# mjoppich/tsxCount

Hardware: AMD Instinct MI355X
Metric: k-mers/sec inserted, k=31, 1e9 synthetic k-mers, 1/2/4/8 GPU; --check pass (higher is better)
Workload: dtype u64

## Files before the change

### tsxcount_amd/csrc/tsx_partition.h

```cpp
#pragma once
#include "tsx_kernels.h"
#include "tsx_layout.h"
#include <type_traits>

namespace tsx {

constexpr int PART_NT = 256;
constexpr int RING_NT = 512;
constexpr int PART_WPT = 4;
constexpr int PART_FLUSH = 16;

template <int RW>
__device__ __forceinline__ void load_rec(const uint64_t *ptr, uint64_t (&r)[RW]) {
    if constexpr (RW == 1) {
        r[0] = *ptr;
    } else {
#pragma unroll
        for (int t = 0; t < RW; t += 2) {
            const uint4 v = *reinterpret_cast<const uint4 *>(ptr + t);
            r[t] = (uint64_t)v.x | ((uint64_t)v.y << 32);
            r[t + 1] = (uint64_t)v.z | ((uint64_t)v.w << 32);
        }
    }
}
template <int RW>
__device__ __forceinline__ void store_rec(uint64_t *ptr, const uint64_t (&r)[RW]) {
    if constexpr (RW == 1) {
        *ptr = r[0];
    } else {
#pragma unroll
        for (int t = 0; t < RW; t += 2)
            *reinterpret_cast<uint4 *>(ptr + t) = make_uint4((uint32_t)r[t], (uint32_t)(r[t] >> 32), (uint32_t)r[t + 1],
                                                             (uint32_t)(r[t + 1] >> 32));
    }
}

constexpr uint32_t OVF_N = 64;
constexpr uint64_t OVF_SALT = 0x5DEECE66D1CE4E5BULL;

__device__ __forceinline__ uint64_t format_record(const TableParams &p, uint64_t key) {
    const uint32_t q1 = ((uint32_t)key + 1u) & (uint32_t)p.seg_mask;
    return ((key >> p.lg) << p.R) | ((uint64_t)q1 << (p.R + p.F));
}

constexpr int PART_MAX_PIECES = 512;
constexpr int PART_ITER = 3;
template <int RW> struct SpillState {
    static constexpr uint32_t DCH_MAX = (RW == 4) ? 48 : 96;
    uint64_t ovk[OVF_N * RW];
    unsigned long long dch[DCH_MAX];
    uint32_t ovc[OVF_N];
    uint32_t ovr[OVF_N];
    uint32_t ovn;
    uint32_t dn;
    uint32_t skew;
};
#define TSX_LDS __attribute__((address_space(3)))
template <int RW>
__device__ __forceinline__ void spill_record(const TableParams *pk, TSX_LDS SpillState<RW> *sp, uint64_t *ovq, uint32_t ovq_cap,
                                             uint32_t dch, RecVal<RW> r, uint32_t d) {
    sp->skew = 1u;
    const uint64_t kk = r.w[0] ^ OVF_SALT;
    if (kk != 0) {
// ... 367 lines not shown
                    if (homeless) spill(cur[q]);
                }
            }
        };
        if constexpr (SKEW) {
            if (s_sp.skew != 0u) append(std::true_type{});
            else append(std::false_type{});
        } else {
            append(std::false_type{});
        }
        lds_barrier();
        flush(false, [&]() {
            __builtin_amdgcn_s_waitcnt(0x0F70);
#pragma unroll
            for (int q = 0; q < RPT; ++q)
#pragma unroll
                for (int t = 0; t < RW; ++t) cur[q][t] = nxt[q][t];
        });
        lds_barrier();
        bc = bn;
    }
    flush(true, []() {});
    lds_barrier();
    {
        const uint32_t dn = SKEW ? s_sp.dn : 0u;
        if (dch && dn % dch != 0u && (dn - 1u) / dch < SpillState<RW>::DCH_MAX) {
            const unsigned long long first = s_sp.dch[(dn - 1u) / dch] - 1ULL;
            if (first + dch <= pk->defer.cap)
                for (uint32_t o = dn % dch + tid; o < dch; o += NT) pk->defer.cnt[first + o] = 0ULL;
        }
    }
    if (dst_cnt)
        for (uint32_t b = tid; b < nb; b += NT) {
            const uint64_t li = dst_bm ? ((uint64_t)b * dst_nr + dst_r0 + r) * cpr + c : ((uint64_t)r * nb + b) * cpr + c;
            dst_cnt[li] = (min(s_cur[b], s_lim[b]) - li * dst_cap * RW) / RW;
        }
    if (tid < OVF_N && s_sp.ovc[tid]) {
        uint64_t rec[RW];
#pragma unroll
        for (int t = 0; t < RW; ++t) rec[t] = s_sp.ovk[tid * RW + t];
        rec[0] ^= OVF_SALT;
        defer_append<RW>(pk, rec, s_sp.ovc[tid]);
    }
    if (tid == 0 && ovq_cnt) ovq_cnt[blockIdx.x] = min(s_sp.ovn, ovq_cap);
    for (int d = 32; d > 0; d >>= 1) spilled += __shfl_down(spilled, d, 64);
    if ((tid & 63) == 0 && spilled) atomicAdd(&p.stats[ST_FALLBACK], (unsigned long long)spilled);
    if (key_sum) {
        for (int d = 32; d > 0; d >>= 1) ksum += __shfl_down(ksum, d, 64);
        if ((tid & 63) == 0 && ksum) atomicAdd(key_sum, ksum);
    }
}

constexpr int SP_NT = 512;
constexpr uint32_t SP_CAPBITS = 5;

__global__ __launch_bounds__(1024) void desc_prefix_kernel(const unsigned long long *cnt, uint32_t nregions,
                                                           unsigned long long *offs, unsigned long long *total,
                                                           uint64_t desc_cap, uint64_t out_cap, unsigned long long *stats) {
    __shared__ unsigned long long s_w[16];
    const uint32_t tid = threadIdx.x, per = (nregions + 1023u) / 1024u;
    unsigned long long sum = 0, lost = 0;
    for (uint32_t i = 0; i < per; ++i) {
        const uint32_t r = tid * per + i;
        if (r < nregions) { sum += min((unsigned long long)cnt[r], (unsigned long long)desc_cap); lost += cnt[r] > desc_cap ? cnt[r] - desc_cap : 0ULL; }
    }
    const unsigned long long inc = wave_incl_scan64(sum);
    if ((tid & 63) == 63) s_w[tid >> 6] = inc;
    __syncthreads();
    unsigned long long base = inc - sum;
    for (uint32_t w = 0; w < (tid >> 6); ++w) base += s_w[w];
    for (uint32_t i = 0; i < per; ++i) {
        const uint32_t r = tid * per + i;
        if (r < nregions) { offs[r] = base; base += min((unsigned long long)cnt[r], (unsigned long long)desc_cap); }
    }
    if (lost && stats) atomicAdd(&stats[ST_FAIL], lost);
    if (tid == 1023) {
        if (base > out_cap) { if (stats) atomicAdd(&stats[ST_FAIL], base - out_cap); base = out_cap; }
        total[0] = base;
    }
}
__global__ __launch_bounds__(256) void desc_pack_kernel(const uint4 *desc, uint64_t desc_cap, const unsigned long long *cnt,
                                                        const unsigned long long *offs, uint32_t nregions, uint4 *out,
                                                        uint64_t out_cap, uint32_t du) {
    for (uint32_t r = blockIdx.x; r < nregions; r += gridDim.x) {
        const uint64_t n = min((uint64_t)cnt[r], desc_cap) * du, o = offs[r] * du;
        const uint4 *src = desc + (uint64_t)r * desc_cap * du;
        for (uint64_t i = threadIdx.x; i < n; i += 256)
            if (o + i < out_cap) out[o + i] = src[i];
    }
}

template <int NT, bool CANON = false, bool LOCAL = false>
__global__ __launch_bounds__(NT, 4) void walk_part_kernel(TableParams p, const uint4 *desc, uint64_t desc_cap,
                                                            const unsigned long long *desc_cnt, uint32_t nregions,
                                                            uint64_t *dst, uint64_t dst_cap, unsigned long long *dst_cnt,
                                                            uint32_t nb, uint32_t shift, uint64_t *ovq_all,
                                                            uint32_t *ovq_cnt, uint32_t ovq_cap, uint64_t n_packed,
                                                            uint32_t dst_g0, uint32_t dst_gtot, int own_flags,
                                                            unsigned long long *emit_sum, int long_desc, uint32_t flush_q,
                                                            int dst_wgm) {
    const int own_only = LOCAL ? 0 : own_flags & 3;
    const bool append = !LOCAL && (own_flags & 4) != 0;
    if constexpr (LOCAL) { n_packed = 0; dst_g0 = 0; long_desc = 0; }
    constexpr int HOT_N = 8;
    __shared__ uint64_t s_hot_key[(NT / 64) * HOT_N];
    __shared__ uint32_t s_hot_cnt[(NT / 64) * HOT_N];
    __shared__ uint64_t s_roll[CANON ? 128 : 64];
    __shared__ uint64_t s_lut4[256];
    uint64_t *const s_mroll = s_roll + 64;
    __shared__ uint64_t s_homh[4];
    __shared__ uint32_t s_njobs[2];
    __shared__ uint32_t s_ovn;
    __shared__ uint64_t s_ovk[OVF_N];
    __shared__ uint32_t s_ovc[OVF_N];
    extern __shared__ uint64_t s_part[];
    constexpr uint32_t CAP = 1u << SP_CAPBITS, cmask = CAP - 1;
    uint64_t *s_stage = s_part;
    unsigned long long *s_meta = reinterpret_cast<unsigned long long *>(s_part + ((size_t)nb << SP_CAPBITS));
    unsigned long long *s_th = s_meta + nb;
    uint32_t *s_cur = reinterpret_cast<uint32_t *>(s_th + nb);
    uint32_t *s_job = s_cur + nb;

    const uint32_t tid = threadIdx.x, lane = tid & 63, wave = tid >> 6;
    const uint32_t wg = blockIdx.x;
    const uint32_t cap32 = (uint32_t)min(dst_cap, (uint64_t)0xFFFFFFF0u);
    const uint32_t gl = dst_g0 + wg;
    const SubListOrder ord = sublist_order(nb, dst_gtot, dst_wgm);
    const uint32_t li0 = sublist_number(ord, 0, gl);
    auto word_of = [&](uint32_t b, uint32_t at) -> uint64_t * { return dst + ((uint64_t)(li0 + b * ord.step_b) * (uint64_t)cap32 + at); };
    auto is_mine = [&](uint64_t hk) -> bool {
        if constexpr (LOCAL) return true;
        if (own_only != 1) return true;
        const uint64_t h1[1] = {hk};
        return owner_shard<1>(p, h1) == p.shard;
    };
    if (tid < 64) s_roll[tid] = p.roll[tid];
    if (tid < 256) s_lut4[tid] = p.roll[64 + tid];
    if (CANON && tid < 64) s_mroll[tid] = p.roll[MROLL1_AT + tid];
    if (tid < 4) {
        const uint64_t x = (0x5555555555555555ULL * (uint64_t)tid) & p.top_mask;
        uint64_t hh = 0;
        for (int grp = 0; grp < 16; ++grp) hh ^= p.roll[64 + grp * 16 + ((x >> (4 * grp)) & 15u)];
        if constexpr (CANON) {
            const uint64_t xc = (0x5555555555555555ULL * (uint64_t)(3 - tid)) & p.top_mask;
            uint64_t hc = 0;
            for (int grp = 0; grp < 16; ++grp) hc ^= p.roll[64 + grp * 16 + ((xc >> (4 * grp)) & 15u)];
            hh = min(hh, hc);
        }
        s_homh[tid] = hh;
    }
    if (tid < (NT / 64) * HOT_N) { s_hot_key[tid] = 0; s_hot_cnt[tid] = 0; }
    if (tid < OVF_N) { s_ovk[tid] = 0; s_ovc[tid] = 0; }
    if (tid < 2) s_njobs[tid] = 0;
    if (tid == 0) s_ovn = (append && ovq_cnt) ? ovq_cnt[blockIdx.x] : 0u;
    for (uint32_t b = tid; b < nb; b += NT) { s_cur[b] = append ? (uint32_t)dst_cnt[li0 + b * ord.step_b] : 0u; s_th[b] = 0; }
    uint64_t *ovq = ovq_all ? ovq_all + (size_t)blockIdx.x * ovq_cap : nullptr;
    unsigned long long added = 0;
    unsigned long long emitted = 0;
    uint32_t spilled = 0;
    const uint32_t k = (uint32_t)p.k;
    const uint32_t inc_ws = (2u * k) >> 5, inc_sh = (2u * k) & 31u;
    const bool two_dwords = k > 16u;
    auto first_hash = [&](uint64_t x) -> uint64_t {
        const uint32_t xl = (uint32_t)x, xh = (uint32_t)(x >> 32);
        uint64_t hx = 0;
#pragma unroll
        for (int grp = 0; grp < 8; ++grp) hx ^= s_lut4[grp * 16 + __builtin_amdgcn_ubfe(xl, 4 * grp, 4)];
        if (two_dwords) {
#pragma unroll
            for (int grp = 0; grp < 8; ++grp) hx ^= s_lut4[128 + grp * 16 + __builtin_amdgcn_ubfe(xh, 4 * grp, 4)];
        }
// ... 6 lines not shown
        const uint64_t kk = key ^ OVF_SALT;
        if (kk != 0) {
            const uint32_t slot = (uint32_t)(mix64(key) >> 40) & (OVF_N - 1);
            const unsigned long long old = atomicCAS(reinterpret_cast<unsigned long long *>(&s_ovk[slot]), 0ULL,
                                                     (unsigned long long)kk);
            if (old == 0ULL || old == kk) { atomicAdd(&s_ovc[slot], 1u); return; }
        }
        if (ovq) {
            const uint32_t at = atomicAdd(&s_ovn, 1u);
            if (at < ovq_cap) { ovq[at] = key; return; }
        }
        defer_append1(pk, key, 1);
    };
    uint32_t round = 0;
    auto flush = [&](bool all, bool wait_loads) {
        const uint32_t par = round & 1u;
        ++round;
        if (tid == 0) s_njobs[par ^ 1u] = 0;
        for (uint32_t b = tid; b < nb; b += NT) {
            const unsigned long long th = s_th[b];
            const uint32_t head = (uint32_t)(th >> 32);
            const uint32_t tail = min((uint32_t)th, head + CAP);
            const uint32_t avail = tail - head;
            const uint32_t at = s_cur[b];
            const uint32_t end = (at + avail) & ~(uint32_t)(PART_FLUSH - 1);
            const uint32_t nout = all ? avail : (end > at ? end - at : 0u);
            s_meta[b] = ((unsigned long long)at << 16) | ((unsigned long long)(head & cmask) << 8) | nout;
            s_th[b] = ((unsigned long long)(head + nout) << 32) | tail;
            s_cur[b] = at + nout;
            if (nout) s_job[atomicAdd(&s_njobs[par], 1u)] = b;
        }
        lds_barrier();
        if (wait_loads) __builtin_amdgcn_s_waitcnt(0x0F70);
        const uint32_t oct = tid >> 3, ol = tid & 7;
        const uint32_t njobs = s_njobs[par];
        constexpr int ITER = 2;
        for (uint32_t j0 = 0; j0 < njobs; j0 += ITER * (NT / 8)) {
            unsigned long long meta[ITER];
            uint32_t bj[ITER];
            uint64_t k0[ITER], k1[ITER];
#pragma unroll
            for (int u = 0; u < ITER; ++u) {
                const uint32_t j = j0 + oct + u * (NT / 8);
                bj[u] = (j < njobs) ? s_job[j] : 0u;
            }
#pragma unroll
            for (int u = 0; u < ITER; ++u) {
                const uint32_t j = j0 + oct + u * (NT / 8);
                meta[u] = (j < njobs) ? s_meta[bj[u]] : 0ULL;
            }
#pragma unroll
            for (int u = 0; u < ITER; ++u) {
                const uint32_t nout = (uint32_t)meta[u] & 0xFFu, hd = ((uint32_t)meta[u] >> 8) & 0xFFu;
                const uint64_t *ring = s_stage + (bj[u] << SP_CAPBITS);
                k0[u] = (ol < nout) ? ring[((hd + ol) ^ bj[u]) & cmask] : 0;
                k1[u] = (ol + 8 < nout) ? ring[((hd + ol + 8) ^ bj[u]) & cmask] : 0;
            }
#pragma unroll
            for (int u = 0; u < ITER; ++u) {
                const uint32_t nout = (uint32_t)meta[u] & 0xFFu, hd = ((uint32_t)meta[u] >> 8) & 0xFFu;
                const uint32_t at = (uint32_t)(meta[u] >> 16);
                const uint64_t *ring = s_stage + (bj[u] << SP_CAPBITS);
                uint64_t *out = word_of(bj[u], at);
                if (ol < nout) { if (at + ol < cap32) out[ol] = k0[u]; else spill(k0[u]); }
                if (ol + 8 < nout) { if (at + ol + 8 < cap32) out[ol + 8] = k1[u]; else spill(k1[u]); }
                if (nout > 16)
                    for (uint32_t q = ol + 16; q < nout; q += 8) {
                        const uint64_t w = ring[((hd + q) ^ bj[u]) & cmask];
                        if (at + q < cap32) out[q] = w; else spill(w);
                    }
            }
        }
    };

    lds_barrier();
    for (uint32_t r = blockIdx.x; r < nregions; r += gridDim.x) {
        uint32_t nr;
        if constexpr (LOCAL) nr = (uint32_t)min((uint64_t)desc_cnt[r], desc_cap);
        else nr = n_packed ? (uint32_t)(((uint64_t)r * desc_cap < n_packed) ? min(desc_cap, n_packed - (uint64_t)r * desc_cap) : 0ULL)
                           : (uint32_t)min((uint64_t)desc_cnt[r], desc_cap);
        const uint32_t per = long_desc ? NT / 4 : NT, me = long_desc ? tid >> 2 : tid;
        const uint4 *rd = desc + (uint64_t)r * desc_cap * (long_desc ? 2u : 1u);
        const uint4 z4 = make_uint4(0, 0, 0, 0);
        uint4 dn = z4, dn2 = z4;
        if (me < nr) { if (long_desc) { dn = rd[2u * me]; dn2 = rd[2u * me + 1u]; } else dn = rd[me]; }
        for (uint32_t base = 0; base < nr; base += per) {
            const uint4 d = dn, d2 = dn2;
            if (base + per < nr) {
                dn = z4; dn2 = z4;
                if (base + per + me < nr) {
                    if (long_desc) { dn = rd[2u * (base + per + me)]; dn2 = rd[2u * (base + per + me) + 1u]; }
                    else dn = rd[base + per + me];
                }
            }
            uint32_t cw0 = d.x, cw1 = d.y, cw2 = d.z, vm = d.w & 0xFFFFu;
            if (!LOCAL && long_desc) {
                const uint32_t t = tid & 3u;
                const uint32_t w0 = d.x, w1 = d.y, w2 = d.z, w3 = d.w, w4 = d2.x, w5 = d2.y;
                cw0 = (t == 0u) ? w0 : (t == 1u) ? w1 : (t == 2u) ? w2 : w3;
                cw1 = (t == 0u) ? w1 : (t == 1u) ? w2 : (t == 2u) ? w3 : w4;
                cw2 = (t == 0u) ? w2 : (t == 1u) ? w3 : (t == 2u) ? w4 : w5;
                const uint32_t vw = (t < 2u) ? d2.z : d2.w;
                vm = (vw >> ((t & 1u) * 16u)) & 0xFFFFu;
            }
            const bool wave_has = __ballot(vm != 0u) != 0ULL;
            uint64_t h = 0, hr = 0;
            uint32_t inc = 0, single = 0;
            if (wave_has) {
                const uint64_t lo = (uint64_t)cw0 | ((uint64_t)cw1 << 32), hi = cw2;
                if (vm) {
                    const uint64_t x = lo & p.top_mask;
                    h = first_hash(x);
                    if constexpr (CANON) {
                        const uint64_t xa[1] = {x};
                        uint64_t r[1];
// ... 44 lines not shown
                        if constexpr (!LOCAL) emitted += tot;
                        const uint64_t key = s_homh[b];
                        uint64_t *hkey = s_hot_key + wave * HOT_N;
                        uint32_t *hcnt = s_hot_cnt + wave * HOT_N;
                        int at = -1;
                        for (int q = 0; q < HOT_N; ++q)
                            if (hcnt[q] && hkey[q] == key) { at = q; break; }
                        if (at < 0)
                            for (int q = 0; q < HOT_N; ++q)
                                if (!hcnt[q]) { at = q; hkey[q] = key; break; }
                        if (at >= 0 && (uint64_t)hcnt[at] + tot < 0xFFFFFFF0ULL) hcnt[at] += tot;
                        else defer_append1(pk, key, tot);
                    }
                }
            }
        }
            bool waited = false;
            for (uint32_t j0 = 0; j0 < 16; j0 += 4) {
                const uint32_t s4 = (single >> j0) & 0xFu;
                if (wave_has) {
                    uint64_t hs[4];
#pragma unroll
                    for (int j = 0; j < 4; ++j) {
                        hs[j] = CANON ? min(h, hr) : h;
                        if (j0 + j < 15) {
                            const uint32_t idx = ((uint32_t)h & 3u) | (__builtin_amdgcn_ubfe(cw0, 2u * (j0 + j), 2u) << 2) |
                                                 (__builtin_amdgcn_ubfe(inc, 2u * (j0 + j), 2u) << 4);
                            if constexpr (CANON) hr = mirror_step(p, s_mroll, hr, idx);
                            h = (h >> 2) ^ s_roll[idx];
                        }
                    }
                    uint32_t m4 = s4;
                    if constexpr (!LOCAL) if (own_only) {
                        if (own_only == 1) {
#pragma unroll
                            for (int j = 0; j < 4; ++j)
                                if (((s4 >> j) & 1u) && !is_mine(hs[j])) m4 &= ~(1u << j);
                        }
                        emitted += (unsigned long long)__popc(m4);
                    }
                    if (__ballot(m4 != 0u) != 0ULL) {
                        uint32_t bq[4];
                        unsigned long long sl[4];
#pragma unroll
                        for (int j = 0; j < 4; ++j) {
                            bq[j] = (uint32_t)(hs[j] >> shift) & (nb - 1);
                            sl[j] = ((m4 >> j) & 1u) ? atomicAdd(&s_th[bq[j]], 1ULL) : 0ULL;
                        }
#pragma unroll
                        for (int j = 0; j < 4; ++j) {
                            if ((m4 >> j) & 1u) {
                                const uint32_t b = bq[j];
                                if ((uint32_t)sl[j] - (uint32_t)(sl[j] >> 32) < CAP) {
                                    s_stage[(b << SP_CAPBITS) + (((uint32_t)sl[j] ^ b) & cmask)] = hs[j];
                                } else {
                                    const uint32_t at = atomicAdd(&s_cur[b], 1u);
                                    if (at < cap32) *word_of(b, at) = hs[j];
                                    else spill(hs[j]);
                                }
                            }
                        }
                    }
                }
                if (LOCAL || (((j0 >> 2) + 1u) % flush_q) == 0u) {
                    lds_barrier();
                    flush(false, !waited);
                    waited = true;
                    lds_barrier();
                }
            }
        }
    }
    lds_barrier();
    flush(true, false);
    lds_barrier();
    for (uint32_t b = tid; b < nb; b += NT) dst_cnt[li0 + b * ord.step_b] = min(s_cur[b], cap32);
    if (tid < OVF_N && s_ovc[tid]) defer_append1(pk, s_ovk[tid] ^ OVF_SALT, s_ovc[tid]);
    if (tid == 0 && ovq_cnt) ovq_cnt[blockIdx.x] = min(s_ovn, ovq_cap);
    if (tid < (NT / 64) * HOT_N && s_hot_cnt[tid]) defer_append1(pk, s_hot_key[tid], s_hot_cnt[tid]);
    if constexpr (!LOCAL) if (emit_sum) {
        for (int d = 32; d > 0; d >>= 1) emitted += __shfl_down(emitted, d, 64);
        if (lane == 0 && emitted) atomicAdd(emit_sum, emitted);
    }
    for (int d = 32; d > 0; d >>= 1) { added += __shfl_down(added, d, 64); spilled += __shfl_down(spilled, d, 64); }
    if (lane == 0) {
        if (added) atomicAdd(&p.stats[ST_KMERS], added);
        if (spilled) atomicAdd(&p.stats[ST_FALLBACK], (unsigned long long)spilled);
    }
}

inline bool walk_local_form(int own_flags, uint64_t n_packed, int long_desc, uint32_t flush_q, const void *emit_sum,
                            uint32_t dst_g0) {
    return own_flags == 0 && n_packed == 0 && !long_desc && flush_q == 1u && emit_sum == nullptr && dst_g0 == 0u;
}

template <int WK>
__global__ __launch_bounds__(PART_NT) void overflow_insert_kernel(TableParams p, const uint64_t *ovq_all,
                                                                  const uint32_t *ovq_cnt, uint32_t cap, uint32_t nq) {
    constexpr int RW = RecWords<WK>::value;
    for (uint32_t qi = blockIdx.x; qi < nq; qi += gridDim.x) {
        const uint32_t n = ovq_cnt[qi];
        for (uint32_t i = threadIdx.x; i < n; i += PART_NT) {
            uint64_t h[WK];
#pragma unroll
            for (int t = 0; t < WK; ++t) h[t] = ovq_all[((size_t)qi * cap + i) * RW + t];
            insert_key<WK>(p, h, 1);
        }
    }
}

template <int WK>
__global__ __launch_bounds__(PART_NT) void deferred_insert_kernel(TableParams p, const uint64_t *rec, const uint64_t *cnt,
                                                                  const unsigned long long *n_ptr, uint64_t n_fixed,
                                                                  uint64_t cap) {
    constexpr int RW = RecWords<WK>::value;
    const uint64_t n = min(n_ptr ? (uint64_t)*n_ptr : n_fixed, cap);
    constexpr uint32_t DN = (RW == 1) ? 2048u : (RW == 2) ? 1024u : 512u;
// ... 595 lines not shown
```

### tsxcount_amd/csrc/tsxcount_hip.hip

```cpp
#include "../../include/tsxcount_hip.h"
#include "tsx_kernels.h"
#include "tsx_partition.h"
#include "tsx_minimizer.h"
#include "tsx_inflate.h"
#include "tsx_output.h"
#include "tsx_query.h"
#include "tsx_baserule.h"
#include "tsx_db.h"
#include "tsx_combine.h"
#include "tsx_joint.h"
#include "tsx_het.h"
#include "tsx_bin.h"
#include "tsx_fasta.h"
#include "tsx_trim.h"
#include "tsx_normalize.h"
#include "tsx_sketch.h"
#include "tsx_prefilter.h"
#include "tsx_pairs.h"
#include "tsx_own.h"

#include <mutex>
#include <hip/hip_runtime.h>

#include <algorithm>
// ... 675 lines not shown
        case 2: { constexpr int WKV = 2; CALL; } break; \
        case 3: { constexpr int WKV = 3; CALL; } break; \
        default: { constexpr int WKV = 4; CALL; } break; \
    }
#define DISPATCH_CANON(m, CALL)                                                    \
    if ((m)->canon) { constexpr bool CANV = true; CALL; } else { constexpr bool CANV = false; CALL; }
#define DISPATCH_BR(m, CALL)                                                                                           \
    if ((m)->p.acgt_only || (m)->qmap_cur) { constexpr bool BRV = true; CALL; } else { constexpr bool BRV = false; CALL; }

static inline int rec_words(int wk) { return wk == 3 ? 4 : wk; }

static int max_seg_bits() {
    static int v = 0;
    if (!v) { v = 18; if (const char *e = getenv("TSX_HIP_SLAB_SEGBITS")) v = std::min(18, std::max(9, atoi(e))); }
    return v;
}
static int slab_bits(const tsx_hip_map *m) {
    const TableParams &p = m->p;
    const int nsegbits = p.l - p.S;
    if (nsegbits <= max_seg_bits() || p.wk != 1 || p.W != 1 || p.lg != p.l) return 0;
    return nsegbits - max_seg_bits();
}
static inline bool slab_build_wanted(const tsx_hip_map *m, size_t n) {
    return slab_bits(m) && (m->path == 2 || (m->path == 0 && n * 32 >= m->lay.table_bytes));
}
static bool can_partition(const tsx_hip_map *m) {
    const TableParams &p = m->p;
    const int nsegbits = p.l - p.S;
    if (nsegbits >= 1 && nsegbits <= (p.lg == p.l && p.wk == 1 && p.W == 1 ? max_seg_bits() : 18)) return true;
    const int sb = slab_bits(m);
    return sb >= 1 && sb <= 4;
}

struct RadixBits { int b1, b2; };
static inline RadixBits radix_bits(int nsegbits) {
    const int b1 = std::min(9, (nsegbits <= 8) ? nsegbits : (nsegbits + 1) / 2);
    return RadixBits{b1, nsegbits - b1};
}
static inline uint32_t cpr2_for(int cus, RadixBits rb) {
    if (rb.b2 <= 0) return 1;
    uint32_t c = std::min<uint32_t>(8, std::max<uint32_t>(1, (uint32_t)(cus * 8) / (1u << rb.b1)));
    while (c & (c - 1)) c &= c - 1;
    return c;
}
static uint32_t level2_cpr(const tsx_hip_map *m) { return cpr2_for(m->cus, radix_bits(m->p.l - m->p.S)); }
static inline uint32_t ring_bits(uint32_t nb) {
    const uint32_t mean = std::max<uint32_t>(1, RING_NT * PART_WPT / nb);
    uint32_t bits = 4;
    while ((1u << bits) < PART_FLUSH + 2 * mean && bits < 6) ++bits;
    return bits;
}
static const uint32_t RECV_RING_BITS = 5;
static inline size_t ring_lds_bytes(uint32_t nb, uint32_t bits) { return (size_t)nb * (((size_t)8 << bits) + 36); }
static inline size_t walk_lds_bytes(uint32_t nb1) { return (size_t)nb1 * (((size_t)8 << SP_CAPBITS) + 8 + 8 + 4 + 4); }
static const size_t ONE_WG_LDS = (size_t)80 << 10;

template <typename B>
static int grow(hipStream_t st, B &buf, size_t need) { return buf.reserve(&st, need, need + need / 8 + 4096); }

static int ensure_deferred(tsx_hip_map *m, uint64_t maxrec, hipStream_t st) {
    const int rw = rec_words(m->p.wk);
    if (!m->d_def_n.get()) TSX_TRY(m->d_def_n.alloc(64));
    if (maxrec > ((uint64_t)1 << 30)) maxrec = std::max<uint64_t>((uint64_t)1 << 28, maxrec / 16);
    if (maxrec <= m->def_cap()) return TSX_HIP_OK;
    const size_t cap = maxrec + maxrec / 8 + 4096;
    int rc = m->d_def_rec.reserve(&st, (size_t)maxrec * rw * 8, cap * rw * 8);
    if (rc == TSX_HIP_OK) rc = m->d_def_cnt.alloc(cap * 8);
    if (rc != TSX_HIP_OK) { m->d_def_rec.reset(); m->d_def_cnt.reset(); }
    return rc;
}

template <typename... K>
static int set_max_lds(int bytes, K... kernels) {
    for (const void *f : {(const void *)kernels...})
        HIP_TRY(hipFuncSetAttribute(f, hipFuncAttributeMaxDynamicSharedMemorySize, bytes));
    return TSX_HIP_OK;
}
template <int RW>
static int set_ring_lds(int bytes) {
    return set_max_lds(bytes, partition_ring_kernel<RW>, partition_ring_kernel<RW, 1024>, partition_ring_kernel<RW, RING_NT, true>,
                       partition_ring_kernel<RW, 1024, true>);
}
template <int NTV>
static int set_walk_lds(int bytes) {
    return set_max_lds(bytes, walk_part_kernel<NTV>, walk_part_kernel<NTV, true>, walk_part_kernel<NTV, false, true>,
                       walk_part_kernel<NTV, true, true>);
}
static int set_partition_attrs(tsx_hip_map *m) {
    if (m->attr_done) return TSX_HIP_OK;
    const int big = 150 << 10, seg = (128 << 10) + (32 << 10);
    TSX_TRY(set_ring_lds<1>(big)); TSX_TRY(set_ring_lds<2>(big)); TSX_TRY(set_ring_lds<4>(big));
    TSX_TRY(set_walk_lds<SP_NT>(big)); TSX_TRY(set_walk_lds<1024>(big));
    TSX_TRY(set_max_lds(seg, build_segments_stream_kernel<false>, build_segments_stream_kernel<true>,
                        build_segments_wide_stream_kernel<1>, build_segments_wide_stream_kernel<2>,
                        build_segments_wide_stream_kernel<3>, build_segments_wide_stream_kernel<4>));
    TSX_TRY(set_max_lds(64 << 10, walk_log_wide_kernel<3>, walk_log_wide_kernel<4>, walk_log_wide_kernel<3, true>,
                        walk_log_wide_kernel<4, true>));
    m->attr_done = true;
    return TSX_HIP_OK;
}

static int plan_partition(tsx_hip_map *m, uint64_t maxrec, int g, bool own_log, uint32_t hist_nb_override,
                          hipStream_t st, PartPlan &pl, int fused_g = 0) {
    const TableParams &p = m->p;
    const int nsegbits = p.l - p.S;
    pl.g = g;
    pl.rw = rec_words(p.wk);
    pl.nseg = 1u << nsegbits;
    const RadixBits rb = radix_bits(nsegbits);
    pl.b1 = rb.b1; pl.b2 = rb.b2;
    pl.nb1 = 1u << pl.b1; pl.nb2 = 1u << pl.b2;
    pl.hist_nb = hist_nb_override ? hist_nb_override : pl.nb1;
    auto even = [](uint64_t v) { return (v + 1) & ~1ULL; };
    pl.log_cap = even(maxrec / g + maxrec / g / 3 + 2048);
    if (const char *e = getenv("TSX_HIP_LOG_CAP")) pl.log_cap = even(std::max(16, atoi(e)));
    pl.cpr2 = cpr2_for(m->cus, rb);
    if (pl.b2) if (const char *e = getenv("TSX_HIP_CPR2")) pl.cpr2 = (uint32_t)std::min(8, std::max(1, atoi(e)));
    const uint64_t per_sub = maxrec / pl.nseg / pl.cpr2;
    pl.cap_sub = (per_sub + per_sub / 4 + 6 * (uint64_t)std::sqrt((double)per_sub + 1.0) + 64 + 15) & ~15ULL;
    pl.fused = fused_g > 0 && pl.b2 > 0 && p.wk == 1 && (fused_g + pl.cpr2 - 1) / pl.cpr2 <= (uint32_t)PART_MAX_PIECES;
    pl.G1 = pl.fused ? (uint32_t)fused_g : 0;
    pl.cap1 = 0;
    pl.l1_wgm = false;
    if (pl.fused) {
        const uint64_t per1 = maxrec / pl.nb1 / pl.G1;
        pl.cap1 = (per1 + per1 / 4 + 6 * (uint64_t)std::sqrt((double)per1 + 1.0) + 64 + 15) & ~15ULL;
        if (const char *e = getenv("TSX_HIP_CAP1")) pl.cap1 = (uint64_t)std::max(16, atoi(e) & ~15);
    }
    const uint64_t rec_cap = pl.fused ? 0 : (own_log ? (uint64_t)g * pl.log_cap : maxrec);
    const size_t need0 = std::max<uint64_t>(own_log ? rec_cap : 0, pl.b2 ? (uint64_t)pl.nseg * pl.cpr2 * pl.cap_sub : 0) * 8 * pl.rw;
    const size_t need1 = (pl.fused ? (uint64_t)pl.nb1 * pl.G1 * pl.cap1 : rec_cap) * 8 * pl.rw;
    TSX_TRY(grow(st, m->d_buf[0], need0));
    TSX_TRY(grow(st, m->d_buf[1], need1));
    pl.buf1 = m->d_buf[1].get();
    const uint32_t hb = std::max(pl.nb1, pl.hist_nb);
    pl.cnt_need = 2 * (size_t)g + 2 * (size_t)hb + (size_t)pl.nseg * pl.cpr2 + (size_t)pl.nb1 * pl.G1;
    const size_t mat = (size_t)hb * g;
    TSX_TRY(grow(st, m->d_cnt, pl.cnt_need * 8 + mat * 12 + 64));
    pl.c_log = m->d_cnt.get();
    pl.c_rstart = pl.c_log + g;
    pl.c_bstart = pl.c_rstart + g; pl.c_bcnt = pl.c_bstart + hb; pl.c_seg = pl.c_bcnt + hb;
    pl.c_l1 = pl.c_seg + (size_t)pl.nseg * pl.cpr2;
    pl.d_offs = pl.c_l1 + (size_t)pl.nb1 * pl.G1;
    pl.d_hist = reinterpret_cast<uint32_t *>(pl.d_offs + mat);
    HIP_TRY(hipMemsetAsync(m->d_cnt.get(), 0, pl.cnt_need * 8, st));
    TSX_TRY(set_partition_attrs(m));
    return TSX_HIP_OK;
}

struct WalkPartLaunch {
    uint32_t grid = 0;
    const uint4 *desc = nullptr; uint64_t desc_cap = 0; const unsigned long long *desc_cnt = nullptr; uint32_t nregions = 0;
    uint64_t *dst = nullptr; uint64_t dst_cap = 0; unsigned long long *dst_cnt = nullptr; uint32_t nb = 0, shift = 0;
    uint64_t *ovq_all = nullptr; uint32_t *ovq_cnt = nullptr; uint32_t ovq_cap = 0; uint64_t n_packed = 0;
    uint32_t dst_g0 = 0, dst_gtot = 0; int own_flags = 0; unsigned long long *emit_sum = nullptr; int long_desc = 0; uint32_t flush_q = 0;
    int dst_wgm = 0;
};
static void launch_walk_part(tsx_hip_map *m, hipStream_t st, const TableParams &pp, WalkPartLaunch &a) {
    const size_t lds = walk_lds_bytes(a.nb);
#define TSX_WALK(NTV, CANV, LOCV)                                                                                              \
    hipLaunchKernelGGL((walk_part_kernel<NTV, CANV, LOCV>), dim3(a.grid), dim3(NTV), lds, st, pp, a.desc, a.desc_cap,          \
                       a.desc_cnt, a.nregions, a.dst, a.dst_cap, a.dst_cnt, a.nb, a.shift, a.ovq_all, a.ovq_cnt, a.ovq_cap,    \
                       a.n_packed, a.dst_g0, a.dst_gtot, a.own_flags, a.emit_sum, a.long_desc, a.flush_q, a.dst_wgm)
    const bool local = walk_local_form(a.own_flags, a.n_packed, a.long_desc, a.flush_q, a.emit_sum, a.dst_g0);
    a.dst_wgm = local ? 1 : 0;
    if (lds > ONE_WG_LDS) {
        if (local) { DISPATCH_CANON(m, TSX_WALK(1024, CANV, true)); } else { DISPATCH_CANON(m, TSX_WALK(1024, CANV, false)); }
    } else {
        if (local) { DISPATCH_CANON(m, TSX_WALK(SP_NT, CANV, true)); } else { DISPATCH_CANON(m, TSX_WALK(SP_NT, CANV, false)); }
    }
#undef TSX_WALK
}

#define DISPATCH_RW(rw, CALL)                        \
    switch (rw) {                                    \
        case 1: { constexpr int RWV = 1; CALL; } break; \
        case 2: { constexpr int RWV = 2; CALL; } break; \
        default: { constexpr int RWV = 4; CALL; } break; \
    }

struct RingLaunch {
    uint32_t grid = 0;
    int rw = 1;
    bool skew = false;
    bool fixed_nt = false;
    const uint64_t *src = nullptr; const unsigned long long *src_start = nullptr, *src_cnt = nullptr; uint64_t src_cap = 0;
    uint32_t nregions = 0, cpr = 1; uint64_t *dst = nullptr; const unsigned long long *offs = nullptr, *offs_base = nullptr;
    unsigned long long *dst_cnt = nullptr; uint64_t dst_cap = 0; uint32_t nb = 0, shift = 0, capbits = 0;
    uint64_t *ovq_all = nullptr; uint32_t *ovq_cnt = nullptr; uint32_t ovq_cap = 0;
    const unsigned long long *src_pcnt = nullptr; uint32_t src_np = 0; uint64_t src_pcap = 0;
    int src_wgm = 0;
    int dst_bm = 0;
    unsigned long long *key_sum = nullptr; uint32_t dst_r0 = 0, dst_nr = 0; int fmt = 0; uint32_t dch = 0; const uint32_t *skew_flag = nullptr;
};
static void launch_ring(hipStream_t st, const TableParams &pp, const RingLaunch &a) {
    const size_t lds = ring_lds_bytes(a.nb, a.capbits);
#define TSX_RING(RWV, NTV, SK)                                                                                                 \
    hipLaunchKernelGGL((partition_ring_kernel<RWV, NTV, SK>), dim3(a.grid), dim3(NTV), lds, st, pp, a.src, a.src_start,        \
                       a.src_cnt, a.src_cap, a.nregions, a.cpr, a.dst, a.offs, a.offs_base, a.dst_cnt, a.dst_cap, a.nb,        \
                       a.shift, a.capbits, a.ovq_all, a.ovq_cnt, a.ovq_cap, a.src_pcnt, a.src_np, a.src_pcap, a.src_wgm,       \
                       a.dst_bm, a.key_sum, a.dst_r0, a.dst_nr, a.fmt, a.dch, a.skew_flag)
    if (!a.fixed_nt && lds > ONE_WG_LDS) {
        if (a.skew) { DISPATCH_RW(a.rw, TSX_RING(RWV, 1024, true)); } else { DISPATCH_RW(a.rw, TSX_RING(RWV, 1024, false)); }
    } else {
        if (a.skew) { DISPATCH_RW(a.rw, TSX_RING(RWV, RING_NT, true)); } else { DISPATCH_RW(a.rw, TSX_RING(RWV, RING_NT, false)); }
    }
#undef TSX_RING
}

struct WalkLogLaunch {
    uint32_t grid = 0;
    const uint4 *desc = nullptr; uint64_t desc_cap = 0; const unsigned long long *desc_cnt = nullptr; uint32_t nregions = 0;
    uint64_t *log = nullptr; uint64_t log_cap = 0; unsigned long long *log_cnt = nullptr; uint32_t *hist = nullptr;
    uint32_t hist_nb = 0, hist_shift = 0; uint64_t n_packed = 0; int long_desc = 0, own_only = 0; unsigned long long *emit_sum = nullptr;
};
static void launch_walk_log(tsx_hip_map *m, hipStream_t st, const TableParams &pp, const WalkLogLaunch &a) {
    const size_t lut_bytes = m->lut.size() * 8;
#define TSX_WALK_WIDE(WKV)                                                                                                     \
    DISPATCH_CANON(m, hipLaunchKernelGGL((walk_log_wide_kernel<WKV, CANV>), dim3(a.grid), dim3(NT), lut_bytes, st, pp, a.desc, \
                                         a.desc_cap, a.desc_cnt, a.nregions, a.log, a.log_cap, a.log_cnt, a.hist, a.hist_nb,   \
                                         a.hist_shift))
    switch (m->p.wk) {
// ... 231 lines not shown
static void launch_strip_desc(tsx_hip_map *m, int grid, hipStream_t st, const TableParams &pp, const PieceText &t, uint4 *desc,
                              uint64_t desc_cap, unsigned long long *desc_cnt, unsigned long long *kmer_sum, int long_desc) {
    DISPATCH_BR(m, hipLaunchKernelGGL((strip_desc_kernel<false, BRV>), dim3(grid), dim3(NT), 0, st, pp, t.text, t.n, t.own_end,
                                      t.head_open, (const uint32_t *)m->d_tile.get(), t.ntiles, desc, desc_cap, desc_cnt, kmer_sum,
                                      long_desc, (unsigned long long *)nullptr, m->qmap_cur));
}

static int describe_piece(tsx_hip_map *m, const PieceText &t, const DescOut &dsc, Event *ev, hipStream_t st) {
    const uint64_t ntiles = t.ntiles;
    const int gdd = (int)std::min<uint64_t>(ntiles, (uint64_t)m->cus * 8), gdr = gdd * (NT / 64);
    const uint32_t du = dsc.long_desc ? 2u : 1u;
    const uint64_t dcap = ((ntiles + gdd - 1) / gdd) * (dsc.long_desc ? 16 : 64);
    TSX_TRY(grow(st, m->d_buf[1], (size_t)gdr * dcap * du * 16));
    TSX_TRY(grow(st, m->d_desc_cnt, ((size_t)2 * gdr + 16) * 8 + (size_t)MZ_MAX_RANKS * m->cus * MZ_WG_PER_CU * 4 + 64));
    unsigned long long *d_cnt = m->d_desc_cnt.get(), *d_offs = d_cnt + gdr, *d_tot = d_offs + gdr;
    uint4 *regions = (uint4 *)m->d_buf[1].get();
    if (dsc.owners) {
        unsigned long long *d_hom = d_cnt + 2 * (size_t)gdr + 8 + ((size_t)MZ_MAX_RANKS * m->cus * MZ_WG_PER_CU + 1) / 2;
        HIP_TRY(hipMemsetAsync(d_hom, 0, 32, st));
        hipLaunchKernelGGL(strip_desc_kernel<true>, dim3(gdd), dim3(NT), 0, st, m->p, t.text, t.n, t.own_end, t.head_open,
                           (const uint32_t *)m->d_tile.get(), ntiles, regions, dcap, d_cnt, dsc.sum, 0, d_hom);
        HIP_TRY(hipGetLastError());
        m->mz_regions = (uint32_t)gdr; m->mz_dcap = dcap;
        return timing_close_parked(m, ev, EV_SCAN_END, st);
    }
    launch_strip_desc(m, gdd, st, m->p, t, regions, dcap, d_cnt, dsc.sum, dsc.long_desc);
    hipLaunchKernelGGL(desc_prefix_kernel, dim3(1), dim3(1024), 0, st, (const unsigned long long *)d_cnt, (uint32_t)gdr,
                       d_offs, d_tot, dcap, (uint64_t)dsc.cap, m->p.stats);
    hipLaunchKernelGGL(desc_pack_kernel, dim3(std::min(gdr, m->cus * 8)), dim3(256), 0, st, (const uint4 *)regions, dcap,
                       (const unsigned long long *)d_cnt, (const unsigned long long *)d_offs, (uint32_t)gdr, dsc.out,
                       dsc.cap * du, du);
    HIP_TRY(hipGetLastError());
    HIP_TRY(hipMemcpyAsync(dsc.count, d_tot, 8, hipMemcpyDeviceToDevice, st));
    return timing_close_parked(m, ev, EV_SCAN_END, st);
}

static int count_piece_atomic(tsx_hip_map *m, const PieceText &t, Event *ev, hipStream_t st) {
    TSX_TRY(ensure_zeroed(m, st));
    const size_t lut_bytes = m->lut.size() * 8;
    const int g3 = (int)std::min<uint64_t>(t.ntiles, (uint64_t)m->cus * 3);
    if (m->pf_armed) {
        DISPATCH_BR(m, DISPATCH_CANON(m, DISPATCH_WK(m, hipLaunchKernelGGL((count_fastq_kernel<WKV, CANV, BRV, true>), dim3(g3), dim3(NT),
                                                            lut_bytes, st, m->p, t.text, t.n, t.own_end, t.head_open,
                                                            (const uint32_t *)m->d_tile.get(), t.ntiles, m->qmap_cur, m->pf_view()))));
    } else {
        DISPATCH_BR(m, DISPATCH_CANON(m, DISPATCH_WK(m, hipLaunchKernelGGL((count_fastq_kernel<WKV, CANV, BRV>), dim3(g3), dim3(NT),
                                                            lut_bytes, st, m->p, t.text, t.n, t.own_end, t.head_open,
                                                            (const uint32_t *)m->d_tile.get(), t.ntiles, m->qmap_cur))));
    }
    HIP_TRY(hipGetLastError());
    return timing_close(ev, EV_SCAN_END, st);
}

static int scan_fused(tsx_hip_map *m, const PieceText &t, PartPlan &pl, const TableParams &pp, int gd, hipStream_t st) {
    const int gdreg = gd * (NT / 64);
    const uint32_t nq2 = pl.nb1 * pl.cpr2;
    TSX_TRY(ensure_ovq(m, (size_t)nq2 + pl.G1, pl.rw, st));
    const char *ll_env = getenv("TSX_HIP_LOCAL_LONG");
    const int lng = ll_env ? (atoi(ll_env) != 0) : 0;
    const uint64_t desc_cap = ((t.ntiles + gd - 1) / gd) * (lng ? 16 : 64);
    TSX_TRY(grow(st, m->d_buf[0], (size_t)gdreg * desc_cap * (lng ? 32 : 16)));
    launch_strip_desc(m, gd, st, pp, t, (uint4 *)m->d_buf[0].get(), desc_cap, pl.c_log, nullptr, lng);
    HIP_TRY(hipGetLastError());
    WalkPartLaunch w;
    w.grid = pl.G1;
    w.desc = (const uint4 *)m->d_buf[0].get(); w.desc_cap = desc_cap; w.desc_cnt = pl.c_log; w.nregions = (uint32_t)gdreg;
    w.dst = pl.buf1; w.dst_cap = pl.cap1; w.dst_cnt = pl.c_l1;
    w.nb = pl.nb1; w.shift = (uint32_t)(m->p.l - pl.b1);
    w.ovq_all = m->d_ovq.get() + (size_t)nq2 * OVQ_CAP; w.ovq_cnt = m->d_ovq_cnt.get() + nq2; w.ovq_cap = OVQ_CAP;
    w.dst_gtot = pl.G1; w.long_desc = lng; w.flush_q = 1u;
    launch_walk_part(m, st, pp, w);
    pl.l1_wgm = w.dst_wgm != 0;
    m->l1_seen = L1Seen{(size_t)(pl.c_l1 - m->d_cnt.get()), pl.nb1, pl.G1, pl.cpr2, pl.cap1, w.dst_wgm};
    return TSX_HIP_OK;
}

static int scan_key_log(tsx_hip_map *m, const PieceText &t, PartPlan &pl, const TableParams &pp, int gs, int gd,
                        uint32_t hist_nb, uint32_t hist_shift, hipStream_t st) {
    const int wk = m->p.wk, gdreg = gd * (NT / 64);
    const int du = (2 * wk + 2 + 3) / 4;
    const uint64_t desc_cap = ((t.ntiles + gd - 1) / gd) * 64;
    TSX_TRY(grow(st, m->d_buf[1], (size_t)gdreg * desc_cap * du * 16));
    pl.buf1 = m->d_buf[1].get();
    TSX_TRY(grow(st, m->d_desc_cnt, (size_t)gdreg * 8));
    uint4 *regions = (uint4 *)m->d_buf[1].get();
#define TSX_DESC_WIDE(WKV)                                                                                                     \
    DISPATCH_BR(m, hipLaunchKernelGGL((strip_desc_wide_kernel<WKV, BRV>), dim3(gd), dim3(NT), 0, st, pp, t.text, t.n, t.own_end, \
                                      t.head_open, (const uint32_t *)m->d_tile.get(), t.ntiles, regions, desc_cap,            \
                                      m->d_desc_cnt.get(), m->qmap_cur))
    switch (wk) {
        case 1:
            launch_strip_desc(m, gd, st, pp, t, regions, desc_cap, m->d_desc_cnt.get(), nullptr, 0);
            HIP_TRY(hipGetLastError());
            break;
        case 2: TSX_DESC_WIDE(2); break;
        case 3: TSX_DESC_WIDE(3); break;
        default: TSX_DESC_WIDE(4); break;
    }
#undef TSX_DESC_WIDE
    WalkLogLaunch w;
    w.grid = (uint32_t)gs;
    w.desc = regions; w.desc_cap = desc_cap; w.desc_cnt = m->d_desc_cnt.get(); w.nregions = (uint32_t)gdreg;
    w.log = m->d_buf[0].get(); w.log_cap = pl.log_cap; w.log_cnt = pl.c_log;
    w.hist = pl.d_hist; w.hist_nb = hist_nb; w.hist_shift = hist_shift;
    launch_walk_log(m, st, pp, w);
    return TSX_HIP_OK;
}

static int split_by_owner(tsx_hip_map *m, const PartPlan &pl, int greg, uint32_t nown, const ShardOut &sh, hipStream_t st) {
    if ((uint64_t)greg * pl.log_cap > sh.send_cap || (sh.own && (uint64_t)greg * pl.log_cap > sh.own_cap)) return TSX_HIP_ERANGE;
    hipLaunchKernelGGL(offsets_rows_kernel, dim3(nown), dim3(1024), 0, st, (const uint32_t *)pl.d_hist, pl.d_offs,
                       (uint32_t)greg, pl.c_bcnt);
    hipLaunchKernelGGL(offsets_finish_kernel, dim3(1), dim3(1024), 0, st, nown, pl.c_bstart, pl.c_bcnt);
    hipLaunchKernelGGL(split_owner_kernel, dim3(std::min(greg, m->cus * 8)), dim3(PART_NT), 0, st,
                       (const uint64_t *)m->d_buf[0].get(), (const unsigned long long *)pl.c_log, pl.log_cap,
                       (uint32_t)greg, sh.send, (const unsigned long long *)pl.d_offs,
                       (const unsigned long long *)pl.c_bstart, (const unsigned long long *)pl.c_bcnt, nown,
                       (uint32_t)m->p.l, sh.own, m->p.shard, sh.key_sum);
    HIP_TRY(hipGetLastError());
    HIP_TRY(hipMemcpyAsync(sh.counts, pl.c_bcnt, nown * sizeof(unsigned long long), hipMemcpyDeviceToDevice, st));
    return TSX_HIP_OK;
}

static int count_piece_partitioned(tsx_hip_map *m, const PieceText &t, const ShardOut &sh, const HotOut &hot, Event *ev,
                                   hipStream_t st) {
    const TableParams &p = m->p;
    const uint64_t own_end = t.own_end, ntiles = t.ntiles;
    const bool sharded = sh.send != nullptr;
    const uint64_t maxrec = (p.line_mask == 3 ? own_end / 2 : own_end) + 65536;
    const uint32_t nown = 1u << (p.lg - p.l);
    const int scan_wgs = (p.wk == 1) ? SCAN_WG_PER_CU : (p.wk == 2 ? 6 : 3);
    const int gs = (int)std::min<uint64_t>(ntiles, (uint64_t)m->cus * scan_wgs);
    const int greg = gs * (NT / 64);
    PartPlan pl;
    const char *fuse_env = getenv("TSX_HIP_FUSE");
    const int fuse = (fuse_env && atoi(fuse_env) == 0) ? 0 : 2;
    const int g_sp = (int)std::min<uint64_t>((own_end + 8191) / 8192, (uint64_t)m->cus * 2);
    const int desc_wgs = 8;
    const int gd = (int)std::min<uint64_t>(ntiles, (uint64_t)m->cus * desc_wgs), gdreg = gd * (NT / 64);
    const bool want_fuse = fuse && !sharded && p.wk == 1;

    int rc = plan_partition(m, maxrec, (want_fuse && fuse == 2) ? std::max(greg, gdreg) : greg, true, sharded ? nown : 0, st,
                            pl, want_fuse ? g_sp : 0);
    if (rc == TSX_HIP_OK && want_fuse && !pl.fused)
        rc = plan_partition(m, maxrec, greg, true, 0, st, pl, 0);
    if (rc != TSX_HIP_OK) return rc;
    TableParams pp = m->p;
    if (sharded) {
        pp.defer = DeferList{hot.keys, hot.cnts, hot.n, hot.cap};
    } else {
        TSX_TRY(ensure_deferred(m, maxrec, st));
        HIP_TRY(hipMemsetAsync(m->d_def_n.get(), 0, 8, st));
        pp.defer = m->defer();
    }
    if (pl.fused) { TSX_TRY(scan_fused(m, t, pl, pp, gd, st)); }
    else { TSX_TRY(scan_key_log(m, t, pl, pp, gs, gd, sharded ? nown : pl.nb1, (uint32_t)(sharded ? p.l : p.l - pl.b1), st)); }
    HIP_TRY(hipGetLastError());
    if (ev) TSX_TRY(timing_record(ev, EV_SCAN_END, EV_PART, st));
    if (sharded) {
        TSX_TRY(split_by_owner(m, pl, greg, nown, sh, st));
        return timing_close_parked(m, ev, EV_PART, st);
    }
    TSX_TRY(run_partition_build(m, pl, m->d_buf[0].get(), nullptr, pl.log_cap, st, ev));
    return timing_close(ev, EV_END, st);
}

static int run_fastq_piece(tsx_hip_map *m, const uint8_t *d_text, uint64_t n, uint64_t own_end, int head_open,
                           hipStream_t st, ShardOut sh = ShardOut(), HotOut hot = HotOut(), DescOut dsc = DescOut()) {
    if (own_end == 0) return TSX_HIP_OK;
    const bool describe = dsc.out || dsc.owners;
    if (m->pf_armed && (sh.send || describe)) return TSX_HIP_EINVAL;
    const PieceText t{d_text, n, own_end, head_open, (own_end + TILE - 1) / TILE};
    TSX_TRY(ensure_tiles(m, t.ntiles, st));
    Event *ev = nullptr;
    TSX_TRY(timing_open(m, ev, st));
    TSX_TRY(line_pass(m, d_text, n, own_end, head_open, st));
    if (ev) TSX_TRY(timing_record(ev, EV_SCAN, EV_SCAN, st));
    if (describe) return describe_piece(m, t, dsc, ev, st);
    const bool use_part = !m->pf_armed && (sh.send || (can_partition(m) && !slab_bits(m) &&
                                         (m->path == 2 || (m->path == 0 && own_end * 32 >= m->lay.table_bytes))));
    return use_part ? count_piece_partitioned(m, t, sh, hot, ev, st) : count_piece_atomic(m, t, ev, st);
}

template <class ArgTests>
static int exch_entry(tsx_hip_map *m, void *stream, hipStream_t &st, ArgTests args_rc) {
    if (exch_refused(m)) return TSX_HIP_EINVAL;
    if (!m) return TSX_HIP_EINVAL;
    m->used = true;
    TSX_TRY(args_rc());
    HIP_TRY(hipSetDevice(m->device));
// ... 4363 lines not shown
```

Baseline: 90.10 billion.

## Deepen local walk staging rings to 64 words with one 1024-thread WG per CU

Adds a template parameter for the per-bucket LDS ring depth in the partition walk kernel. The local walk path now uses 64-word rings when they fit in the LDS budget, launched as one 1024-thread workgroup per CU with a smaller grid, and flushes every two quarters instead of every quarter. The intent is fewer, larger coalesced flushes to global sublists and fewer barrier/flush rounds. The cost is half the resident workgroups per CU and a changed grid size for the fused partition plan.

```diff
diff --git a/tsxcount_amd/csrc/tsx_partition.h b/tsxcount_amd/csrc/tsx_partition.h
--- a/tsxcount_amd/csrc/tsx_partition.h
+++ b/tsxcount_amd/csrc/tsx_partition.h
@@ -9,6 +9,8 @@
 constexpr int RING_NT = 512;
 constexpr int PART_WPT = 4;
 constexpr int PART_FLUSH = 16;
+constexpr uint32_t RING_DEPTH32 = 5, RING_DEPTH64 = 6;
+constexpr uint32_t local_flush_quarters(uint32_t capbits) { return capbits >= RING_DEPTH64 ? 2u : 1u; }
 
 template <int RW>
 __device__ __forceinline__ void load_rec(const uint64_t *ptr, uint64_t (&r)[RW]) {
@@ -482,7 +484,6 @@
 }
 
 constexpr int SP_NT = 512;
-constexpr uint32_t SP_CAPBITS = 5;
 
 __global__ __launch_bounds__(1024) void desc_prefix_kernel(const unsigned long long *cnt, uint32_t nregions,
                                                            unsigned long long *offs, unsigned long long *total,
@@ -520,7 +521,7 @@
     }
 }
 
-template <int NT, bool CANON = false, bool LOCAL = false>
+template <int NT, bool CANON = false, bool LOCAL = false, uint32_t CAPBITS = RING_DEPTH32>
 __global__ __launch_bounds__(NT, 4) void walk_part_kernel(TableParams p, const uint4 *desc, uint64_t desc_cap,
                                                             const unsigned long long *desc_cnt, uint32_t nregions,
                                                             uint64_t *dst, uint64_t dst_cap, unsigned long long *dst_cnt,
@@ -544,9 +545,12 @@
     __shared__ uint64_t s_ovk[OVF_N];
     __shared__ uint32_t s_ovc[OVF_N];
     extern __shared__ uint64_t s_part[];
-    constexpr uint32_t CAP = 1u << SP_CAPBITS, cmask = CAP - 1;
+    static_assert(CAPBITS == RING_DEPTH32 || CAPBITS == RING_DEPTH64, "ring depth: 32 or 64 words");
+    constexpr uint32_t CAP = 1u << CAPBITS, cmask = CAP - 1;
+    static_assert(CAP <= 0xFFu, "s_meta keeps head & cmask and nout (<= CAP) in 8 bits each");
+    constexpr uint32_t LOCAL_FLUSH_Q = local_flush_quarters(CAPBITS);
     uint64_t *s_stage = s_part;
-    unsigned long long *s_meta = reinterpret_cast<unsigned long long *>(s_part + ((size_t)nb << SP_CAPBITS));
+    unsigned long long *s_meta = reinterpret_cast<unsigned long long *>(s_part + ((size_t)nb << CAPBITS));
     unsigned long long *s_th = s_meta + nb;
     uint32_t *s_cur = reinterpret_cast<uint32_t *>(s_th + nb);
     uint32_t *s_job = s_cur + nb;
@@ -659,7 +663,7 @@
 #pragma unroll
             for (int u = 0; u < ITER; ++u) {
                 const uint32_t nout = (uint32_t)meta[u] & 0xFFu, hd = ((uint32_t)meta[u] >> 8) & 0xFFu;
-                const uint64_t *ring = s_stage + (bj[u] << SP_CAPBITS);
+                const uint64_t *ring = s_stage + (bj[u] << CAPBITS);
                 k0[u] = (ol < nout) ? ring[((hd + ol) ^ bj[u]) & cmask] : 0;
                 k1[u] = (ol + 8 < nout) ? ring[((hd + ol + 8) ^ bj[u]) & cmask] : 0;
             }
@@ -667,7 +671,7 @@
             for (int u = 0; u < ITER; ++u) {
                 const uint32_t nout = (uint32_t)meta[u] & 0xFFu, hd = ((uint32_t)meta[u] >> 8) & 0xFFu;
                 const uint32_t at = (uint32_t)(meta[u] >> 16);
-                const uint64_t *ring = s_stage + (bj[u] << SP_CAPBITS);
+                const uint64_t *ring = s_stage + (bj[u] << CAPBITS);
                 uint64_t *out = word_of(bj[u], at);
                 if (ol < nout) { if (at + ol < cap32) out[ol] = k0[u]; else spill(k0[u]); }
                 if (ol + 8 < nout) { if (at + ol + 8 < cap32) out[ol + 8] = k1[u]; else spill(k1[u]); }
@@ -818,7 +822,7 @@
                             if ((m4 >> j) & 1u) {
                                 const uint32_t b = bq[j];
                                 if ((uint32_t)sl[j] - (uint32_t)(sl[j] >> 32) < CAP) {
-                                    s_stage[(b << SP_CAPBITS) + (((uint32_t)sl[j] ^ b) & cmask)] = hs[j];
+                                    s_stage[(b << CAPBITS) + (((uint32_t)sl[j] ^ b) & cmask)] = hs[j];
                                 } else {
                                     const uint32_t at = atomicAdd(&s_cur[b], 1u);
                                     if (at < cap32) *word_of(b, at) = hs[j];
@@ -828,7 +832,7 @@
                         }
                     }
                 }
-                if (LOCAL || (((j0 >> 2) + 1u) % flush_q) == 0u) {
+                if (LOCAL ? (((j0 >> 2) + 1u) % LOCAL_FLUSH_Q) == 0u : (((j0 >> 2) + 1u) % flush_q) == 0u) {
                     lds_barrier();
                     flush(false, !waited);
                     waited = true;
diff --git a/tsxcount_amd/csrc/tsxcount_hip.hip b/tsxcount_amd/csrc/tsxcount_hip.hip
--- a/tsxcount_amd/csrc/tsxcount_hip.hip
+++ b/tsxcount_amd/csrc/tsxcount_hip.hip
@@ -751,8 +751,13 @@
 }
 static const uint32_t RECV_RING_BITS = 5;
 static inline size_t ring_lds_bytes(uint32_t nb, uint32_t bits) { return (size_t)nb * (((size_t)8 << bits) + 36); }
-static inline size_t walk_lds_bytes(uint32_t nb1) { return (size_t)nb1 * (((size_t)8 << SP_CAPBITS) + 8 + 8 + 4 + 4); }
+static inline size_t walk_lds_bytes(uint32_t nb1, uint32_t bits) { return (size_t)nb1 * (((size_t)8 << bits) + 8 + 8 + 4 + 4); }
 static const size_t ONE_WG_LDS = (size_t)80 << 10;
+static const size_t RING_LDS_MAX = (size_t)150 << 10;
+
+static const int LOCAL_WALK_NT = 1024;
+static inline bool local_walk_deep(uint32_t nb1) { return walk_lds_bytes(nb1, RING_DEPTH64) <= RING_LDS_MAX; }
+static inline int walk_wgs_per_cu(uint32_t nb1, bool local) { return (local && local_walk_deep(nb1)) ? 1 : 2; }
 
 template <typename B>
 static int grow(hipStream_t st, B &buf, size_t need) { return buf.reserve(&st, need, need + need / 8 + 4096); }
@@ -780,6 +785,10 @@
     return set_max_lds(bytes, partition_ring_kernel<RW>, partition_ring_kernel<RW, 1024>, partition_ring_kernel<RW, RING_NT, true>,
                        partition_ring_kernel<RW, 1024, true>);
 }
+static int set_deep_lds(int bytes) {
+    return set_max_lds(bytes, walk_part_kernel<LOCAL_WALK_NT, false, true, RING_DEPTH64>,
+                       walk_part_kernel<LOCAL_WALK_NT, true, true, RING_DEPTH64>);
+}
 template <int NTV>
 static int set_walk_lds(int bytes) {
     return set_max_lds(bytes, walk_part_kernel<NTV>, walk_part_kernel<NTV, true>, walk_part_kernel<NTV, false, true>,
@@ -787,9 +796,9 @@
 }
 static int set_partition_attrs(tsx_hip_map *m) {
     if (m->attr_done) return TSX_HIP_OK;
-    const int big = 150 << 10, seg = (128 << 10) + (32 << 10);
+    const int big = (int)RING_LDS_MAX, seg = (128 << 10) + (32 << 10);
     TSX_TRY(set_ring_lds<1>(big)); TSX_TRY(set_ring_lds<2>(big)); TSX_TRY(set_ring_lds<4>(big));
-    TSX_TRY(set_walk_lds<SP_NT>(big)); TSX_TRY(set_walk_lds<1024>(big));
+    TSX_TRY(set_walk_lds<SP_NT>(big)); TSX_TRY(set_walk_lds<1024>(big)); TSX_TRY(set_deep_lds(big));
     TSX_TRY(set_max_lds(seg, build_segments_stream_kernel<false>, build_segments_stream_kernel<true>,
                         build_segments_wide_stream_kernel<1>, build_segments_wide_stream_kernel<2>,
                         build_segments_wide_stream_kernel<3>, build_segments_wide_stream_kernel<4>));
@@ -856,17 +865,20 @@
     int dst_wgm = 0;
 };
 static void launch_walk_part(tsx_hip_map *m, hipStream_t st, const TableParams &pp, WalkPartLaunch &a) {
-    const size_t lds = walk_lds_bytes(a.nb);
-#define TSX_WALK(NTV, CANV, LOCV)                                                                                              \
-    hipLaunchKernelGGL((walk_part_kernel<NTV, CANV, LOCV>), dim3(a.grid), dim3(NTV), lds, st, pp, a.desc, a.desc_cap,          \
+    const bool local = walk_local_form(a.own_flags, a.n_packed, a.long_desc, a.flush_q, a.emit_sum, a.dst_g0);
+    const bool deep = local && local_walk_deep(a.nb);
+    const size_t lds = walk_lds_bytes(a.nb, deep ? RING_DEPTH64 : RING_DEPTH32);
+#define TSX_WALK(NTV, CANV, LOCV, BITS)                                                                                        \
+    hipLaunchKernelGGL((walk_part_kernel<NTV, CANV, LOCV, BITS>), dim3(a.grid), dim3(NTV), lds, st, pp, a.desc, a.desc_cap,    \
                        a.desc_cnt, a.nregions, a.dst, a.dst_cap, a.dst_cnt, a.nb, a.shift, a.ovq_all, a.ovq_cnt, a.ovq_cap,    \
                        a.n_packed, a.dst_g0, a.dst_gtot, a.own_flags, a.emit_sum, a.long_desc, a.flush_q, a.dst_wgm)
-    const bool local = walk_local_form(a.own_flags, a.n_packed, a.long_desc, a.flush_q, a.emit_sum, a.dst_g0);
     a.dst_wgm = local ? 1 : 0;
-    if (lds > ONE_WG_LDS) {
-        if (local) { DISPATCH_CANON(m, TSX_WALK(1024, CANV, true)); } else { DISPATCH_CANON(m, TSX_WALK(1024, CANV, false)); }
+    if (deep) {
+        DISPATCH_CANON(m, TSX_WALK(LOCAL_WALK_NT, CANV, true, RING_DEPTH64));
+    } else if (lds > ONE_WG_LDS) {
+        if (local) { DISPATCH_CANON(m, TSX_WALK(1024, CANV, true, RING_DEPTH32)); } else { DISPATCH_CANON(m, TSX_WALK(1024, CANV, false, RING_DEPTH32)); }
     } else {
-        if (local) { DISPATCH_CANON(m, TSX_WALK(SP_NT, CANV, true)); } else { DISPATCH_CANON(m, TSX_WALK(SP_NT, CANV, false)); }
+        if (local) { DISPATCH_CANON(m, TSX_WALK(SP_NT, CANV, true, RING_DEPTH32)); } else { DISPATCH_CANON(m, TSX_WALK(SP_NT, CANV, false, RING_DEPTH32)); }
     }
 #undef TSX_WALK
 }
@@ -1204,12 +1216,16 @@
     return timing_close(ev, EV_SCAN_END, st);
 }
 
+static bool local_long_descriptions() {
+    const char *e = getenv("TSX_HIP_LOCAL_LONG");
+    return e && atoi(e) != 0;
+}
+
 static int scan_fused(tsx_hip_map *m, const PieceText &t, PartPlan &pl, const TableParams &pp, int gd, hipStream_t st) {
     const int gdreg = gd * (NT / 64);
     const uint32_t nq2 = pl.nb1 * pl.cpr2;
     TSX_TRY(ensure_ovq(m, (size_t)nq2 + pl.G1, pl.rw, st));
-    const char *ll_env = getenv("TSX_HIP_LOCAL_LONG");
-    const int lng = ll_env ? (atoi(ll_env) != 0) : 0;
+    const int lng = local_long_descriptions() ? 1 : 0;
     const uint64_t desc_cap = ((t.ntiles + gd - 1) / gd) * (lng ? 16 : 64);
     TSX_TRY(grow(st, m->d_buf[0], (size_t)gdreg * desc_cap * (lng ? 32 : 16)));
     launch_strip_desc(m, gd, st, pp, t, (uint4 *)m->d_buf[0].get(), desc_cap, pl.c_log, nullptr, lng);
@@ -1287,7 +1303,9 @@
     PartPlan pl;
     const char *fuse_env = getenv("TSX_HIP_FUSE");
     const int fuse = (fuse_env && atoi(fuse_env) == 0) ? 0 : 2;
-    const int g_sp = (int)std::min<uint64_t>((own_end + 8191) / 8192, (uint64_t)m->cus * 2);
+    const bool walk_local = !local_long_descriptions();
+    const int g_sp = (int)std::min<uint64_t>((own_end + 8191) / 8192,
+                                             (uint64_t)m->cus * walk_wgs_per_cu(1u << radix_bits(p.l - p.S).b1, walk_local));
     const int desc_wgs = 8;
     const int gd = (int)std::min<uint64_t>(ntiles, (uint64_t)m->cus * desc_wgs), gdreg = gd * (NT / 64);
     const bool want_fuse = fuse && !sharded && p.wk == 1;
```

Result: faster. 91.47 billion (median of 6 runs) (+1.5%).
